# ljubobratovicrelja/tensor-truth

Measured on AMD Instinct MI355X. Metric: queries/sec (embed+top-k+rerank) over 10M x 1024 corpus, higher is better.
Workload: dtype bf16

## Files before the change

### tensor-truth_amd/csrc/encoder.h

```cpp
#pragma once
#include "common.h"

enum { TT_EPI_BIAS = 0, TT_EPI_GELU = 1, TT_EPI_RESIDUAL = 2, TT_EPI_TANH = 3, TT_EPI_QKV = 4,
       TT_EPI_VT = 5 ,
       TT_EPI_SCAN = 6  };

struct GemmParams {
    const uint16_t* A;
    const uint16_t* W;
    const float* bias;
    const uint16_t* residual;
    uint16_t* C;
    uint16_t* vt;
    int M, N, K, lda, ldc, ldr, ldvt, vt_col0;
    const float* a_scale;
    const float* w_scale;
    int fp8;
    uint8_t* C8;
    float c8_inv_scale;
    int nt_store;
    int sn;
    int xp;
    int32_t* scan_cnt;
    float* scan_scores;
    int32_t* scan_idx;
    int scan_cap;
    int32_t scan_idx_base;
    float* scan_dense;
    int scan_dense_stride;
    int scan_tile_stride;
    int scan_rows;
    int x3;
    int ldw;
    int c_lo_off;
    float* C32;
    const float* res32;
    const uint16_t* res_planes;
    int res_lo_off;
    uint16_t* vt_lo;
    int x3_zero_lo;
    int xc;
    const uint8_t* a_scales;
    const uint8_t* w_scales;
    uint8_t* c_scales;
#if TT_DIAG
    int lnf;
    const float* lnf_rows;
    const float* lnf_c0;
    const float* lnf_c1;
    float* lnf_part;
#endif
};
int tt_scan_gemm_launch(const uint16_t* corpus, int64_t rows, int dim, const uint16_t* queries256, const float* thr256,
                        int32_t* cnt, float* cand_scores, int32_t* cand_idx, int cap, int32_t idx_base, hipStream_t st);
int tt_scan_gemm_sample_launch(const uint16_t* corpus, int tiles, int tile_stride, int dim, const uint16_t* queries256, const float* thr256,
// ... 98 lines not shown
```

### tensor-truth_amd/csrc/gemm.hip

```cpp
#include "common.h"
#include <type_traits>

#include "encoder.h"
#include "f16c.h"

namespace {

constexpr int BM = 128, BN = 128, BK = 64;
constexpr int kGemmThreads = 256;
constexpr int kTileBytes = BM * BK * 2;
constexpr int kStageBytes = 2 * kTileBytes;
constexpr int kGemmLds = 2 * kStageBytes;

__device__ __forceinline__ f32x2 gelu_erf2(f32x2 x) {
    const f32x2 u = f32x2{fabsf(x.x), fabsf(x.y)};
    f32x2 q = u * -9.697845371e-07f + 4.016999810e-05f;
    q = q * u + -7.211678312e-04f;
    q = q * u + 7.490924560e-03f;
    q = q * u + -5.142170191e-02f;
    q = q * u + -4.614778757e-01f;
    q = q * u + -1.149914980e+00f;
    q = q * u + -1.000091195e+00f;
    const f32x2 e = f32x2{__builtin_amdgcn_exp2f(q.x), __builtin_amdgcn_exp2f(q.y)};
    const f32x2 r = f32x2{fmaxf(x.x, 0.f), fmaxf(x.y, 0.f)};
// ... 920 lines not shown
                    }
                }
        }
}

#define TT_SLOT_END()                                         \
    do {                                                      \
        __builtin_amdgcn_sched_barrier(0);                    \
        __builtin_amdgcn_s_barrier();                         \
        __builtin_amdgcn_sched_barrier(0);                    \
    } while (0)

typedef int v8i __attribute__((ext_vector_type(8)));
struct Frag2 { ex8 lo, hi; };
__device__ __forceinline__ f32x4 mfma_fp8(const ex8& a0, const ex8& a1, const ex8& b0, const ex8& b1, f32x4 c) {
    const v8i a = __builtin_bit_cast(v8i, Frag2{a0, a1});
    const v8i b = __builtin_bit_cast(v8i, Frag2{b0, b1});
    return __builtin_amdgcn_mfma_scale_f32_16x16x128_f8f6f4(a, b, c, 0, 0, 0, 0x7F7F7F7F, 0, 0x7F7F7F7F);
}

constexpr int kXcScaleOff = kLds3;
constexpr int kLdsXc = kLds3 + 2 * 8192;
__device__ __forceinline__ void glds4(const void* base, uint32_t voff, uint32_t lds_addr) {
    asm volatile("s_mov_b32 m0, %2\n\ts_nop 0\n\tglobal_load_lds_dword %0, %1"
                 :: "v"(voff), "s"(base), "s"(lds_addr) : "memory", "m0");
}
template <int OA, int OB>
__device__ __forceinline__ f32x4 mfma_fp8_scaled(const ex8& a0, const ex8& a1, const ex8& b0, const ex8& b1, f32x4 c, uint32_t scale_a,
                                                 uint32_t scale_b) {
    const v8i a = __builtin_bit_cast(v8i, Frag2{a0, a1});
    const v8i b = __builtin_bit_cast(v8i, Frag2{b0, b1});
    return __builtin_amdgcn_mfma_scale_f32_16x16x128_f8f6f4(a, b, c, 0, 0, OA, (int)scale_a, OB, (int)scale_b);
}
template <int N, class F>
__device__ __forceinline__ void static_for(F&& f) {
    if constexpr (N > 0) {
        static_for<N - 1>(f);
        f(std::integral_constant<int, N - 1>{});
    }
}

template <int EPI, int SLOTS, bool FP8 = false, bool X3 = false, bool XC = false, bool RP = false>
__global__ __launch_bounds__(kThreads3, 2) void gemm_kernel_v3(GemmParams p) {
    static_assert(!(FP8 && X3), "split-bf16 operands are bf16");
    static_assert(!XC || (!FP8 && !X3 && kF16), "f16c operands: the fp16 instantiation, no other operand mode");
    constexpr int ES = FP8 ? 1 : 2;
    extern __shared__ __attribute__((aligned(16))) char smem[];
    const int tid = threadIdx.x;
    const int lane = tid & 63;
    const int wave = __builtin_amdgcn_readfirstlane(tid >> 6);
    const int wm = wave >> 2, wn = wave & 3;

    const int mt_n = p.M / BM3, nt_n = (p.N + BN3 - 1) / BN3;
    int L = blockIdx.x;
    {
        const int nwg = gridDim.x;
        if ((nwg & 7) == 0) L = (L & 7) * (nwg >> 3) + (L >> 3);
    }
    const int SN = p.sn > 0 ? p.sn : (nt_n < 4 ? nt_n : 4);
    const int SM = 32 / SN > 0 ? 32 / SN : 1;
    const int per_super = SM * SN;
    const int supers_n = (nt_n + SN - 1) / SN;
    const int sidx = L / per_super, widx = L % per_super;
    const int tm = (sidx / supers_n) * SM + widx / SN;
    const int tn = (sidx % supers_n) * SN + widx % SN;
    if (tm >= mt_n || tn >= nt_n) return;
    int m0_nominal = tm * BM3;
    if constexpr (EPI == TT_EPI_SCAN) {
        if (p.scan_tile_stride > 1) m0_nominal *= p.scan_tile_stride;
        if (p.scan_rows && m0_nominal + BM3 > p.scan_rows) m0_nominal = p.scan_rows - BM3;
    }
    const int m0 = m0_nominal, n0 = tn * BN3;
    const int nk1 = p.K * ES / 128;
    constexpr int TB = X3 ? 64 : 128;
    const int nk = X3 ? 2 * nk1 : (XC ? 2 * nk1 : nk1);
    auto tile_a = [&](int t) { return t; };
    auto tile_w = [&](int t) { return t; };

    f32x4 acc[2][2][2][4];
#pragma unroll
    for (int a = 0; a < 2; ++a)
#pragma unroll
        for (int b = 0; b < 2; ++b)
#pragma unroll
            for (int c = 0; c < 2; ++c)
#pragma unroll
                for (int d = 0; d < 4; ++d) acc[a][b][c][d] = f32x4{0.f, 0.f, 0.f, 0.f};

    const int frow = lane & 15, fchk = lane >> 4, sw = (frow >> 1) & 7;
    const int off0 = frow * 128 + ((fchk ^ sw) << 4);
    const int off1 = frow * 128 + (((4 + fchk) ^ sw) << 4);
    const int a_row0 = wm * 64 * 128;
    const int w_row0 = wn * 32 * 128;

    uint32_t voffA[2], voffW[2];
#pragma unroll
    for (int j = 0; j < 2; ++j) {
        const int r = 16 * wave + 8 * j + (lane >> 3);
        const int chunk = (lane & 7) ^ ((r >> 1) & 7);
        const uint32_t coff = X3 ? (chunk < 4 ? (uint32_t)chunk * 16u : (uint32_t)p.K * 2u + (uint32_t)(chunk - 4) * 16u) : (uint32_t)chunk * 16u;
        voffA[j] = (uint32_t)r * (uint32_t)p.lda * (uint32_t)ES + coff;
        const int wr = (X3 && n0 + (r >> 5) * 64 + 64 > p.N) ? 0 : w_row_of(r);
        voffW[j] = (uint32_t)wr * (uint32_t)(p.ldw ? p.ldw : p.K) * (uint32_t)ES + coff;
    }

    unsigned long long* dbg0 = reinterpret_cast<unsigned long long*>(p.vt);
    auto cstamp = [&](int slot) {
        if constexpr (SLOTS == 46) {
            if ((int)blockIdx.x == (p.xp >> 20) && tid == 0 && dbg0) dbg0[20 + slot] = __builtin_amdgcn_s_memtime();
            if ((slot == 0 || slot == 3) && tid == 0 && dbg0) {
                unsigned long long* rec = dbg0 + 256 + (size_t)blockIdx.x * 4;
                rec[slot == 0 ? 0 : 1] = __builtin_amdgcn_s_memtime();
                if (slot == 0)
                    rec[2] = ((unsigned long long)__builtin_amdgcn_s_getreg(20 | (31 << 11)) << 32) |
                             (unsigned long long)__builtin_amdgcn_s_getreg(4 | (31 << 11));
            }
        }
    };
    constexpr bool kResLds = (EPI == TT_EPI_RESIDUAL) && !X3 && !XC;
    uint32_t voffR[2] = {0u, 0u};
    if constexpr (kResLds) {
#pragma unroll
        for (int j = 0; j < 2; ++j) {
            const int r16 = 8 * j + (lane >> 3);
            const int c = (lane & 7) ^ ((r16 >> 1) & 7);
            voffR[j] = (uint32_t)r16 * (uint32_t)p.ldr * 2u + (uint32_t)(c * 16);
        }
    }
    auto stage_res = [&](int part) {
        if constexpr (kResLds) {
#pragma unroll
            for (int od = 0; od < 2; ++od) {
                const char* base = reinterpret_cast<const char*>(
                    p.residual + (size_t)(m0 + (part >> 1) * 128 + wm * 64 + ((part & 1) * 2 + od) * 16) * p.ldr + n0 + wn * 64);
                const unsigned long long b64 = reinterpret_cast<unsigned long long>(base);
                const unsigned int blo = __builtin_amdgcn_readfirstlane((unsigned int)b64);
                const unsigned int bhi = __builtin_amdgcn_readfirstlane((unsigned int)(b64 >> 32));
                base = reinterpret_cast<const char*>(((unsigned long long)bhi << 32) | blo);
                char* dst = smem + (res_slot(part) + 4 * od) * kHalf + 2048 * wave;
                const uint32_t lds_dst = (uint32_t)(uintptr_t)(__attribute__((address_space(3))) char*)dst;
#pragma unroll
                for (int j = 0; j < 2; ++j) glds16(base, voffR[j], lds_dst + 1024 * j);
            }
        }
    };

    cstamp(0);
    if constexpr (EPI == TT_EPI_SCAN) {
        if (tid == 0) *reinterpret_cast<int*>(smem + kScanHitOff) = 0;
        if ((p.xp & 0x10000) && lane == 0) *reinterpret_cast<int*>(smem + kScanHitOff + wave * 1024) = 0;
    }
    if (wave == 0) {
        uint32_t boff = lane * 16;
        if constexpr (X3) {
            const uint32_t last = (uint32_t)((p.N - n0 < BN3 ? p.N - n0 : BN3) * 4 - 16);
            boff = boff < last ? boff : last;
        }
        glds16(p.bias + n0, boff, (uint32_t)(uintptr_t)(__attribute__((address_space(3))) char*)smem + kBiasOff);
    }
    if constexpr (FP8 && EPI != TT_EPI_VT) {
        if (wave == 1) glds16(p.a_scale + m0, lane * 16, (uint32_t)(uintptr_t)(__attribute__((address_space(3))) char*)smem + kScaleOff);
        if (wave == 2) glds16(p.w_scale + n0, lane * 16, (uint32_t)(uintptr_t)(__attribute__((address_space(3))) char*)smem + kScaleOff + 1024);
    }
#if TT_DIAG
    if constexpr (!FP8 && !X3 && !XC && (EPI == TT_EPI_BIAS || EPI == TT_EPI_GELU || EPI == TT_EPI_RESIDUAL)) {
        if (p.lnf) {
            const uint32_t l0 = (uint32_t)(uintptr_t)(__attribute__((address_space(3))) char*)smem;
            if (wave == 1) glds16(p.lnf_c0 + n0, lane * 16, l0 + kScaleOff);
            if (wave == 2 && p.lnf == 2) glds16(p.lnf_c1 + n0, lane * 16, l0 + kScaleOff + 1024);
            if (wave == 3) glds16(p.lnf_rows + (size_t)m0 * 2, lane * 16, l0 + kScaleOff + 2048);
            if (wave == 4) glds16(p.lnf_rows + (size_t)(m0 + 128) * 2, lane * 16, l0 + kScaleOff + 3072);
        }
    }
#endif
    stage_half<0, ES>(p, smem, 0, 0, 0, wave, voffA, m0, n0, TB);
    stage_half<1, ES>(p, smem, 0, 0, 0, wave, voffW, m0, n0, TB);
    stage_half<1, ES>(p, smem, 1, 0, 0, wave, voffW, m0, n0, TB);
    stage_half<0, ES>(p, smem, 1, 0, 0, wave, voffA, m0, n0, TB);
    if (nk > 1) {
        stage_half<0, ES>(p, smem, 0, 1, tile_a(1), wave, voffA, m0, n0, TB);
        stage_half<1, ES>(p, smem, 0, 1, tile_w(1), wave, voffW, m0, n0, TB);
    }
    if (nk > 1) {
        asm volatile("s_waitcnt vmcnt(6)" ::: "memory");
    } else {
        asm volatile("s_waitcnt vmcnt(0)" ::: "memory");
    }
    TT_SLOT_END();
    cstamp(1);
    const bool late = wave >= 4;
    if (late) TT_SLOT_END();

    ex8 xf[4][2], wf0[2][2], wf1[2][2];

    auto read_a = [&](const char* base) {
#pragma unroll
        for (int mt = 0; mt < 4; ++mt) {
            xf[mt][0] = *reinterpret_cast<const ex8*>(base + a_row0 + mt * 2048 + off0);
            xf[mt][1] = *reinterpret_cast<const ex8*>(base + a_row0 + mt * 2048 + off1);
        }
    };
    auto read_w = [&](ex8(&wf)[2][2], const char* base) {
#pragma unroll
        for (int nt = 0; nt < 2; ++nt) {
            wf[nt][0] = *reinterpret_cast<const ex8*>(base + w_row0 + nt * 2048 + off0);
            wf[nt][1] = *reinterpret_cast<const ex8*>(base + w_row0 + nt * 2048 + off1);
        }
    };
    uint32_t sa_reg[2] = {0u, 0u}, sw_reg = 0u;
    const int sa_off = (wm * 16 + frow) * 16 + fchk * 4;
    const int sw_off = 1024 + (wn * 16 + frow) * 16 + fchk * 4;
    auto stage_scales = [&](int t) {
        if constexpr (XC) {
            const int u = t - nk1 + (wave >> 1), nks = nk1 >> 1;
            const uint8_t* src = (wave & 1) ? p.w_scales + ((size_t)(n0 >> 8) * nk1 + u) * 1024
                                            : p.a_scales + ((size_t)(m0 >> 8) * nks + (u >= nks ? u - nks : u)) * 1024;
            const unsigned long long b64 = reinterpret_cast<unsigned long long>(src);
            const unsigned int blo = __builtin_amdgcn_readfirstlane((unsigned int)b64);
            const unsigned int bhi = __builtin_amdgcn_readfirstlane((unsigned int)(b64 >> 32));
            const uint32_t dst = (uint32_t)(uintptr_t)(__attribute__((address_space(3))) char*)smem + kXcScaleOff +
                                 (((t - nk1) >> 2) & 1) * 8192 + wave * 1024;
            glds16(reinterpret_cast<const void*>(((unsigned long long)bhi << 32) | blo), (uint32_t)lane * 16u, dst);
        }
    };
    constexpr bool vblk = (EPI == TT_EPI_VT);
    auto mma = [&](f32x4(&c)[2][4], const ex8(&wf)[2][2]) {
        __builtin_amdgcn_s_setprio(1);
        if constexpr (FP8) {
#pragma unroll
            for (int nt = 0; nt < 2; ++nt)
#pragma unroll
                for (int mt = 0; mt < 4; ++mt) {
                    if constexpr (vblk) c[nt][mt] = mfma_fp8(xf[mt][0], xf[mt][1], wf[nt][0], wf[nt][1], c[nt][mt]);
                    else c[nt][mt] = mfma_fp8(wf[nt][0], wf[nt][1], xf[mt][0], xf[mt][1], c[nt][mt]);
                }
        } else if constexpr (X3) {
#pragma unroll
            for (int term = 0; term < 3; ++term) {
                const int sa = term == 2 ? 1 : 0, sw = term == 1 ? 1 : 0;
#pragma unroll
                for (int nt = 0; nt < 2; ++nt)
#pragma unroll
                    for (int mt = 0; mt < 4; ++mt) {
                        if constexpr (vblk) c[nt][mt] = TT_MFMA_16x16x32(xf[mt][sa], wf[nt][sw], c[nt][mt]);
                        else c[nt][mt] = TT_MFMA_16x16x32(wf[nt][sw], xf[mt][sa], c[nt][mt]);
                    }
            }
        } else if constexpr (vblk) {
#pragma unroll
            for (int ss = 0; ss < 2; ++ss)
#pragma unroll
                for (int nt = 0; nt < 2; ++nt)
#pragma unroll
                    for (int mt = 0; mt < 4; ++mt)
                        c[nt][mt] = TT_MFMA_16x16x32(xf[mt][ss], wf[nt][ss], c[nt][mt]);
        } else {
#pragma unroll
            for (int ss = 0; ss < 2; ++ss)
#pragma unroll
                for (int nt = 0; nt < 2; ++nt)
#pragma unroll
                    for (int mt = 0; mt < 4; ++mt)
                        c[nt][mt] = TT_MFMA_16x16x32(wf[nt][ss], xf[mt][ss], c[nt][mt]);
        }
        __builtin_amdgcn_s_setprio(0);
    };
    auto mma8 = [&](f32x4(&c)[2][4], const ex8(&wf)[2][2], uint32_t sa, uint32_t sw, auto qnc) {
        if constexpr (XC) {
            constexpr int QN = decltype(qnc)::value;
            __builtin_amdgcn_s_setprio(1);
            static_for<2>([&](auto ntc) {
                static_for<4>([&](auto mtc) {
                    constexpr int nt = decltype(ntc)::value, mt = decltype(mtc)::value;
                    if constexpr (vblk) c[nt][mt] = mfma_fp8_scaled<mt, QN * 2 + nt>(xf[mt][0], xf[mt][1], wf[nt][0], wf[nt][1], c[nt][mt], sa, sw);
                    else c[nt][mt] = mfma_fp8_scaled<QN * 2 + nt, mt>(wf[nt][0], wf[nt][1], xf[mt][0], xf[mt][1], c[nt][mt], sw, sa);
                });
            });
            __builtin_amdgcn_s_setprio(0);
        }
    };
    unsigned long long* dbg = reinterpret_cast<unsigned long long*>(p.vt);
    int dbg_i = 0;
    auto stamp = [&](int t) {
        if constexpr (SLOTS == 46) {
            if ((int)blockIdx.x == (p.xp >> 20) && t == 6 && (lane == 0) && dbg) {
                __builtin_amdgcn_sched_barrier(0);
                dbg[wave * 32 + dbg_i] = __builtin_amdgcn_s_memtime();
                ++dbg_i;
                __builtin_amdgcn_sched_barrier(0);
            }
        }
    };
    auto wait_n = [&](int n) {
        if (n == 8) asm volatile("s_waitcnt vmcnt(8) lgkmcnt(0)" ::: "memory");
        else if (n == 6) asm volatile("s_waitcnt vmcnt(6) lgkmcnt(0)" ::: "memory");
        else if (n == 9) asm volatile("s_waitcnt vmcnt(9) lgkmcnt(0)" ::: "memory");
        else if (n == 7) asm volatile("s_waitcnt vmcnt(7) lgkmcnt(0)" ::: "memory");
        else asm volatile("s_waitcnt vmcnt(0) lgkmcnt(0)" ::: "memory");
        TT_SLOT_END();
    };
#if TT_DIAG
    const int eabl = (p.xp & 0x80000) ? ((p.xp >> 4) & 15) : 0;
#else
    constexpr int eabl = 0;
#endif
    auto tile4 = [&](int t, auto bufc, auto f8c) {
        constexpr int B = decltype(bufc)::value;
        constexpr bool F8T = XC && decltype(f8c)::value;
        const bool dma_on = !((eabl & 1) && t >= 2), rd_on = !((eabl & 2) && t >= 2);
        const bool more1 = t + 1 < nk && dma_on, more2 = t + 2 < nk && dma_on;
        const int sc_la = (XC && t + 1 >= nk1 && t + 1 < nk && ((t + 1 - nk1) & 3) == 0) ? 1 : 0;
        const int sc_lb = (XC && t + 2 >= nk1 && t + 2 < nk && ((t + 2 - nk1) & 3) == 0) ? 1 : 0;
        const char* sbuf = smem + kXcScaleOff + (((t - nk1) >> 2) & 1) * 8192 + ((t - nk1) & 3) * 2048;
        stamp(t);
        if (more1) {
            stage_half<1, ES>(p, smem, 1, B ^ 1, tile_w(t + 1), wave, voffW, m0, n0, TB);
            stage_half<0, ES>(p, smem, 1, B ^ 1, tile_a(t + 1), wave, voffA, m0, n0, TB);
        } else if (kResLds) {
            stage_res(1);
        }
        stamp(t);
        if (rd_on) {
            read_a(smem + slot_off(0, 0, B));
            read_w(wf0, smem + slot_off(1, 0, B));
            read_w(wf1, smem + slot_off(1, 1, B));
        }
        if constexpr (F8T) {
            sa_reg[0] = *reinterpret_cast<const uint32_t*>(sbuf + sa_off);
            sw_reg = *reinterpret_cast<const uint32_t*>(sbuf + sw_off);
        }
        stamp(t);
        if (SLOTS == 46) asm volatile("s_waitcnt lgkmcnt(0)" ::: "memory");
        stamp(t);
        wait_n((t + 1 < nk || kResLds) ? 8 + sc_la : 0);
        stamp(t);
        if constexpr (F8T) {
            mma8(acc[0][0], wf0, sa_reg[0], sw_reg, std::integral_constant<int, 0>{});
            mma8(acc[0][1], wf1, sa_reg[0], sw_reg, std::integral_constant<int, 1>{});
        } else {
            mma(acc[0][0], wf0);
            mma(acc[0][1], wf1);
        }
        stamp(t);
        TT_SLOT_END();
        stamp(t);
        if (more2) {
            stage_half<0, ES>(p, smem, 0, B, tile_a(t + 2), wave, voffA, m0, n0, TB);
            stage_half<1, ES>(p, smem, 0, B, tile_w(t + 2), wave, voffW, m0, n0, TB);
            if (sc_lb) stage_scales(t + 2);
        } else if (kResLds) {
            stage_res(B == 0 ? 0 : 2);
        }
        stamp(t);
        if (rd_on) read_a(smem + slot_off(0, 1, B));
        if constexpr (F8T) sa_reg[1] = *reinterpret_cast<const uint32_t*>(sbuf + 512 + sa_off);
        stamp(t);
        if (SLOTS == 46) asm volatile("s_waitcnt lgkmcnt(0)" ::: "memory");
        stamp(t);
        wait_n((t + 2 < nk || kResLds) ? 6 + sc_lb : 0);
        stamp(t);
        if constexpr (F8T) {
            mma8(acc[1][1], wf1, sa_reg[1], sw_reg, std::integral_constant<int, 1>{});
            mma8(acc[1][0], wf0, sa_reg[1], sw_reg, std::integral_constant<int, 0>{});
        } else {
            mma(acc[1][1], wf1);
            mma(acc[1][0], wf0);
        }
        stamp(t);
        TT_SLOT_END();
        stamp(t);
    };

    if constexpr (XC) {
        for (int t = 0; t < nk1; t += 2) {
            tile4(t, std::integral_constant<int, 0>{}, std::false_type{});
            tile4(t + 1, std::integral_constant<int, 1>{}, std::false_type{});
        }
        for (int t = nk1; t < nk; t += 2) {
            tile4(t, std::integral_constant<int, 0>{}, std::true_type{});
            tile4(t + 1, std::integral_constant<int, 1>{}, std::true_type{});
        }
    } else {
        for (int t = 0; t < nk; t += 2) {
            tile4(t, std::integral_constant<int, 0>{}, std::false_type{});
            if (t + 1 < nk) tile4(t + 1, std::integral_constant<int, 1>{}, std::false_type{});
        }
    }
    cstamp(2);
    if (!late) TT_SLOT_END();
    stage_res(3);

    if constexpr (X3) {
        if (n0 + wn * 64 >= p.N) return;
    }
    if constexpr (vblk) {
#pragma unroll
        for (int qm = 0; qm < 2; ++qm)
#pragma unroll
            for (int qn = 0; qn < 2; ++qn)
                gemm_epilogue_vt<2, 4, FP8, X3>(p, acc[qm][qn], m0 + qm * 128 + wm * 64, n0 + wn * 64 + qn * 32, lane);
    } else if constexpr (X3) {
        epilogue_x3<EPI, RP>(p, acc, smem, kBiasOff, m0, n0, wm, wn, lane);
    } else if constexpr (XC && EPI == TT_EPI_RESIDUAL) {
        epilogue_x3<EPI>(p, acc, smem, kBiasOff, m0, n0, wm, wn, lane);
    } else if constexpr (XC && EPI == TT_EPI_GELU) {
        epilogue_xc<EPI>(p, acc, smem, kBiasOff, m0, n0, wm, wn, lane);
    } else if constexpr (XC && EPI == TT_EPI_BIAS) {
        if (p.c_lo_off) epilogue_h2(p, acc, smem, kBiasOff, m0, n0, wm, wn, lane);
        else epilogue_all<EPI, true, false>(p, acc, smem, kBiasOff, kScaleOff, m0, n0, wm, wn, wave, lane, false, NoNext{});
    } else if constexpr (EPI == TT_EPI_QKV) {
#pragma unroll
        for (int qm = 0; qm < 2; ++qm)
#pragma unroll
            for (int qn = 0; qn < 2; ++qn)
                gemm_epilogue_wide<EPI, 2, 4>(p, acc[qm][qn], m0 + qm * 128 + wm * 64, n0 + wn * 64 + qn * 32, lane);
    } else if constexpr (EPI == TT_EPI_SCAN) {
        if (p.scan_dense) scan_sample_epilogue(p, acc, tm, wm, wn, lane);
        else if (p.xp & 0x10000) scan_filter_epilogue<2>(p, acc, smem, kBiasOff, m0, wm, wn, lane);
        else scan_filter_epilogue<1>(p, acc, smem, kBiasOff, m0, wm, wn, lane);
    } else if constexpr (SLOTS == 47) {
#pragma unroll
        for (int qm = 0; qm < 2; ++qm)
#pragma unroll
            for (int qn = 0; qn < 2; ++qn)
                gemm_epilogue_wide<EPI, 2, 4, true>(p, acc[qm][qn], m0 + qm * 128 + wm * 64, n0 + wn * 64 + qn * 32, lane);
    } else {
        epilogue_all<EPI, true, FP8>(p, acc, smem, kBiasOff, kScaleOff, m0, n0, wm, wn, wave, lane, false, NoNext{}, kScaleOff, kScaleOff + 2048);
    }
    if constexpr (SLOTS == 46) {
        asm volatile("s_waitcnt vmcnt(0)" ::: "memory");
        cstamp(3);
    }
}

template <int EPI, bool FP8 = false, bool STAMP = false>
__global__ __launch_bounds__(kThreads3, 2) void gemm_kernel_p(GemmParams p, int nwg) {
    constexpr int ES = FP8 ? 1 : 2;
    extern __shared__ __attribute__((aligned(16))) char smem[];
    const int tid = threadIdx.x;
    const int lane = tid & 63;
    const int wave = __builtin_amdgcn_readfirstlane(tid >> 6);
    const int wm = wave >> 2, wn = wave & 3;

    const int mt_n = p.M / BM3, nt_n = p.N / BN3;
    const int SN = p.sn > 0 ? p.sn : (nt_n < 4 ? nt_n : 4);
    const int SM = 32 / SN > 0 ? 32 / SN : 1;
    const int per_super = SM * SN;
    const int supers_n = (nt_n + SN - 1) / SN;
    const int nk = p.K * ES / 128;
    auto decode = [&](int v, int& m0, int& n0) {
        const int L = (v & 7) * (nwg >> 3) + (v >> 3);
        const int sidx = L / per_super, widx = L % per_super;
        const int tm = (sidx / supers_n) * SM + widx / SN;
        const int tn = (sidx % supers_n) * SN + widx % SN;
        int mm = tm * BM3;
        if constexpr (EPI == TT_EPI_SCAN) {
            if (p.scan_rows && mm + BM3 > p.scan_rows) mm = p.scan_rows - BM3;
        }
        m0 = __builtin_amdgcn_readfirstlane(mm);
        n0 = __builtin_amdgcn_readfirstlane(tn * BN3);
        return tm < mt_n && tn < nt_n;
    };
    auto next_valid = [&](int v, int& m0, int& n0) {
        for (v += gridDim.x; v < nwg; v += gridDim.x)
// ... 172 lines not shown
        const bool align = (p.xp & 4) == 0;
        if (align && !late) TT_SLOT_END();

        int lane_e = lane;
        asm volatile("" : "+v"(lane_e));
        if constexpr (EPI == TT_EPI_SCAN)
            scan_filter_epilogue<2>(p, acc, smem, kBiasOff + bpar * 1024, m0, wm, wn, lane_e);
        else
            epilogue_all<EPI, false, FP8>(p, acc, smem, kBiasOff + bpar * 1024, kScaleOff + bpar * 2048, m0, n0, wm, wn, wave, lane_e,
                                          false, NoNext{}, kScaleOff + bpar * 1024, kScaleOff + 2048 + bpar * 2048);
        pstamp(101);
        ++tile_no;
        if (!has_next) {
            if (!align && !late) TT_SLOT_END();
            break;
        }
        if (align && late) TT_SLOT_END();
        v = vn; m0 = m1; n0 = n1; bpar ^= 1; first = false;
        vn = next_valid(v, m1, n1);
        has_next = vn < nwg;
    }
}
#undef TT_SLOT_END
}

inline int super_sn(int nt_n) {
    static const int env = TT_DIAG_ENV_INT("TT_GEMM_SN", 0);
    int sn = env > 0 ? env : 4;
    if (sn > nt_n) sn = nt_n;
    while (32 % sn) --sn;
    return sn;
}

inline bool small_grid_v1() {
    static const bool on = TT_DIAG_ENV_INT("TT_GEMM_SMALL_V1", 1) != 0;
    return on;
}

template <int EPI>
int launch_fp8(const GemmParams& p, hipStream_t st) {
    if constexpr (EPI == TT_EPI_BIAS || EPI == TT_EPI_GELU || EPI == TT_EPI_VT || EPI == TT_EPI_RESIDUAL) {
        const int nk = p.K / 128;
        if (EPI == TT_EPI_RESIDUAL && (!p.residual || p.ldr % 8)) {
            tt_set_error("gemm fp8: residual epilogue without residual");
            return TT_E_INVALID;
        }
        if (p.M % v3::BM3 || p.N % v3::BN3 || p.K % 128 || nk < 2 || (nk & 1) || p.ldc % 8 || p.lda % 16 || !p.a_scale || !p.w_scale) {
            tt_set_error("gemm fp8: M=%d N=%d K=%d must be multiples of 256/256/256 with row / column scales", p.M, p.N, p.K);
            return TT_E_UNSUPPORTED;
        }
        const int mt_n = p.M / v3::BM3, nt_n = p.N / v3::BN3;
        const int SN = super_sn(nt_n), SM = 32 / SN;
        const int supers = ((mt_n + SM - 1) / SM) * ((nt_n + SN - 1) / SN);
        int blocks = supers * SM * SN;
        blocks = (blocks + 7) / 8 * 8;
        TT_SET_MAX_LDS((v3::gemm_kernel_v3<EPI, 4, true>), v3::kLds3);
        {
            TtProfScope prof(TT_K_GEMM, st);
            GemmParams q = p;
            q.sn = SN;
            hipLaunchKernelGGL((v3::gemm_kernel_v3<EPI, 4, true>), dim3(blocks), dim3(v3::kThreads3), v3::kLds3, st, q);
        }
        TT_CHECK_LAUNCH();
        return TT_OK;
    } else {
        tt_set_error("gemm fp8: epilogue %d has no fp8 form", EPI);
// ... 508 lines not shown

template <int EPI>
int launch(const GemmParams& p, hipStream_t st) {
    if constexpr (!kF16) if (p.fp8) return launch_fp8<EPI>(p, st);
    static const bool trace = TT_DIAG_ENV_INT("TT_GEMM_TRACE", 0) == 1;
    if (trace) fprintf(stderr, "gemm launch<%d> M=%d N=%d K=%d lda=%d ldc=%d ldr=%d\n", EPI, p.M, p.N, p.K, p.lda, p.ldc, p.ldr);
    static const int variant = TT_DIAG_ENV_INT("TT_GEMM_VARIANT", 5);
    const bool small_grid = EPI != TT_EPI_VT && (long long)(p.M / v3::BM3) * (p.N / v3::BN3) < 128 && small_grid_v1();
    if (variant >= 4 && !small_grid && p.M % v3::BM3 == 0 && p.N % v3::BN3 == 0 && p.ldc % 8 == 0 &&
        (EPI != TT_EPI_RESIDUAL || (p.ldr % 8 == 0 && (p.K / BK) % 2 == 0))) {
        const int mt_n = p.M / v3::BM3, nt_n = p.N / v3::BN3;
        const int SN = super_sn(nt_n), SM = 32 / SN;
        const int supers = ((mt_n + SM - 1) / SM) * ((nt_n + SN - 1) / SN);
        int blocks = supers * SM * SN;
        blocks = (blocks + 7) / 8 * 8;
        static const int xp = TT_DIAG_ENV_INT("TT_GEMM_XP", 0);
        if constexpr (EPI == TT_EPI_GELU || EPI == TT_EPI_BIAS) {
            const int cus = tt_cu_count_cached() / 8 * 8;
            if (variant == 5 && (EPI == TT_EPI_GELU || (xp & 1)) && (p.K / BK) % 2 == 0 && p.K / BK >= 2 && blocks > cus && cus >= 8) {
                constexpr int kLdsP = v3::kLds3 + (TT_DIAG ? 2048 : 0);
                TT_SET_MAX_LDS(v3::gemm_kernel_p<EPI>, kLdsP);
                {
                    TtProfScope prof(TT_K_GEMM, st);
                    GemmParams q = p;
                    q.sn = SN;
                    q.xp = xp;
                    hipLaunchKernelGGL(v3::gemm_kernel_p<EPI>, dim3(cus), dim3(v3::kThreads3), kLdsP, st, q, blocks);
                }
                TT_CHECK_LAUNCH();
                return TT_OK;
            }
        }
        auto kern = v3::gemm_kernel_v3<EPI, 4>;
#if TT_DIAG
        if constexpr (EPI == TT_EPI_BIAS) {
            static const int abl = TT_DIAG_ENV_INT("TT_GEMM_ABLATE", 0);
            if (abl == 8) {
                const int cus8 = tt_cu_count_cached() / 8 * 8;
                TT_SET_MAX_LDS((v3::gemm_kernel_p<EPI, false, true>), v3::kLds3);
                GemmParams q8 = p;
                q8.sn = SN;
                q8.xp = xp;
                hipLaunchKernelGGL((v3::gemm_kernel_p<EPI, false, true>), dim3(cus8), dim3(v3::kThreads3), v3::kLds3, st, q8, blocks);
                TT_CHECK_LAUNCH();
                return TT_OK;
            }
            if (abl == 6) kern = v3::gemm_kernel_v3<EPI, 46>;
            if (abl == 7) kern = v3::gemm_kernel_v3<EPI, 47>;
            if (abl == 6 || abl == 7) TT_CHECK_HIP(hipFuncSetAttribute(reinterpret_cast<const void*>(kern), hipFuncAttributeMaxDynamicSharedMemorySize, v3::kLds3));
        }
#endif
        TT_SET_MAX_LDS((v3::gemm_kernel_v3<EPI, 4>), v3::kLds3);
        GemmParams q = p;
        static const int nts = TT_DIAG_ENV_INT("TT_GEMM_NT_STORE", 1);
        q.nt_store = nts;
        q.sn = SN;
        static const bool a0 = TT_DIAG_ENV_INT("TT_GEMM_DEBUG_A0", 0) == 1;
        if (a0) q.xp |= 0x20000;
        static const bool head_major = TT_DIAG_ENV_INT("TT_GEMM_HEAD_MAJOR", 0) == 1;
        if (head_major) q.xp |= 0x40000;
        static const int stamp_block = TT_DIAG_ENV_INT("TT_GEMM_STAMP_BLOCK", 0);
        q.xp |= stamp_block << 20;
        static const int energy = TT_DIAG_ENV_INT("TT_GEMM_ENERGY", 0);
        if (energy) q.xp |= 0x80000 | ((energy & 15) << 4);
        {
            TtProfScope prof(TT_K_GEMM, st);
            hipLaunchKernelGGL(kern, dim3(blocks), dim3(v3::kThreads3), v3::kLds3, st, q);
        }
        TT_CHECK_LAUNCH();
        return TT_OK;
    }
    if constexpr (EPI == TT_EPI_VT) {
        tt_set_error("gemm: internal V^T epilogue needs the 256x256 kernel");
        return TT_E_UNSUPPORTED;
    }
    const int mt_n = p.M / BM, nt_n = p.N / BN;
    const int SN = nt_n < 8 ? nt_n : 8, SM = 8;
    const int supers = ((mt_n + SM - 1) / SM) * ((nt_n + SN - 1) / SN);
    int blocks = supers * SM * SN;
    blocks = (blocks + 7) / 8 * 8;
    static const int staged16 = TT_DIAG_ENV_INT("TT_GEMM_STAGED16", 1);
    if (staged16 && staged_enabled() && (long long)mt_n * nt_n <= (staged16 > 1 ? staged16 : tt_cu_count_cached()) && p.K % 64 == 0) {
        TT_SET_MAX_LDS((gemm_staged_kernel<EPI, false>), kStagedLds);
        {
            TtProfScope prof(TT_K_GEMM, st);
            hipLaunchKernelGGL((gemm_staged_kernel<EPI, false>), dim3(blocks), dim3(kStagedThreads), kStagedLds, st, p);
        }
        TT_CHECK_LAUNCH();
        return TT_OK;
    }
    auto kern = gemm_kernel<EPI>;
    TT_SET_MAX_LDS(kern, kGemmLds);
    {
        TtProfScope prof(TT_K_GEMM, st);
        hipLaunchKernelGGL(kern, dim3(blocks), dim3(kGemmThreads), kGemmLds, st, p);
    }
    TT_CHECK_LAUNCH();
    return TT_OK;
}

// ... 49 lines not shown
    if ((p.lda % 8) || (p.ldc % 4) || !p.A || !p.W || !p.C || !p.bias) {
        tt_set_error("gemm: bad leading dimension / null pointer");
        return TT_E_INVALID;
    }
    if (skinny_shape(p)) {
        switch (epilogue) {
            case TT_EPI_BIAS: return launch_skinny<TT_EPI_BIAS>(p, st);
            case TT_EPI_GELU: return launch_skinny<TT_EPI_GELU>(p, st);
            case TT_EPI_RESIDUAL:
                if (!p.residual || p.ldr % 4) { tt_set_error("gemm: residual epilogue without residual"); return TT_E_INVALID; }
                return launch_skinny<TT_EPI_RESIDUAL>(p, st);
            case TT_EPI_TANH: return launch_skinny<TT_EPI_TANH>(p, st);
            case TT_EPI_QKV:
                if (!p.vt || p.vt_col0 % 16) { tt_set_error("gemm: qkv epilogue without vt"); return TT_E_INVALID; }
                return launch_skinny<TT_EPI_QKV>(p, st);
            default: tt_set_error("gemm: unknown epilogue %d", epilogue); return TT_E_INVALID;
        }
    }
    if (p.M % BM || p.N % BN || p.K % BK || p.K <= 0) {
        tt_set_error("gemm: M=%d N=%d K=%d must be multiples of %d/%d/%d (or M a multiple of 64 up to 256)", p.M, p.N, p.K, BM, BN, BK);
        return TT_E_UNSUPPORTED;
    }
    switch (epilogue) {
        case TT_EPI_BIAS: return launch<TT_EPI_BIAS>(p, st);
        case TT_EPI_GELU: return launch<TT_EPI_GELU>(p, st);
        case TT_EPI_RESIDUAL:
            if (!p.residual) { tt_set_error("gemm: residual epilogue without residual"); return TT_E_INVALID; }
            return launch<TT_EPI_RESIDUAL>(p, st);
        case TT_EPI_TANH: return launch<TT_EPI_TANH>(p, st);
        case TT_EPI_QKV: {
            if (!p.vt) { tt_set_error("gemm: qkv epilogue without vt"); return TT_E_INVALID; }
            static const int variant = TT_DIAG_ENV_INT("TT_GEMM_VARIANT", 5);
            const int nv = p.N - p.vt_col0;
            static const int split = TT_DIAG_ENV_INT("TT_GEMM_QKV_SPLIT", 1);
            const bool small_grid = (long long)(p.M / v3::BM3) * (p.N / v3::BN3) < 128 && small_grid_v1();
            if (variant >= 3 && split && !small_grid && p.M % v3::BM3 == 0 && p.vt_col0 % v3::BN3 == 0 && nv % v3::BN3 == 0 &&
                nv > 0 && p.ldc % 8 == 0 && p.ldvt % 8 == 0) {
                GemmParams a = p;
                a.N = p.vt_col0;
                if (int rc = launch<TT_EPI_BIAS>(a, st)) return rc;
                GemmParams b = p;
                b.W = p.W + (size_t)p.vt_col0 * p.K;
                b.bias = p.bias + p.vt_col0;
                b.N = nv;
                b.vt_col0 = 0;
                return launch<TT_EPI_VT>(b, st);
            }
            return launch<TT_EPI_QKV>(p, st);
        }
        default: tt_set_error("gemm: unknown epilogue %d", epilogue); return TT_E_INVALID;
    }
}

#ifndef TT_SCAN_PERSIST_DEFAULT
#define TT_SCAN_PERSIST_DEFAULT 1
#endif
int tt_scan_gemm_sample_launch(const uint16_t* corpus, int tiles, int tile_stride, int dim, const uint16_t* queries256, const float* thr256,
                               float* dense, int dense_stride, hipStream_t st) {
    if (tiles <= 0) return TT_OK;
    if constexpr (kF16) { tt_set_error("scan gemm: the corpus is bf16 (bf16 instantiation only)"); return TT_E_UNSUPPORTED; }
    else
    if (dim % 128 || dim <= 0 || tile_stride < 1 || !dense || dense_stride < tiles * 8 || (int64_t)tiles * tile_stride * v3::BM3 > INT32_MAX) {
        tt_set_error("scan gemm sample: tiles=%d stride=%d dim=%d dense_stride=%d", tiles, tile_stride, dim, dense_stride);
        return TT_E_UNSUPPORTED;
    }
    GemmParams p{};
    p.A = corpus;
    p.W = queries256;
    p.bias = thr256;
    p.M = tiles * v3::BM3;
// ... 70 lines not shown
```

Measured before the change: 110.2.

## Walk multiple GEMM tiles per workgroup in the v3 bf16 kernel

```diff
diff --git a/tensor-truth_amd/csrc/encoder.h b/tensor-truth_amd/csrc/encoder.h
--- a/tensor-truth_amd/csrc/encoder.h
+++ b/tensor-truth_amd/csrc/encoder.h
@@ -21,6 +21,7 @@
     int nt_store;
     int sn;
     int xp;
+    int walk, walk_rounds, walk_slots;
     int32_t* scan_cnt;
     float* scan_scores;
     int32_t* scan_idx;
diff --git a/tensor-truth_amd/csrc/gemm.hip b/tensor-truth_amd/csrc/gemm.hip
--- a/tensor-truth_amd/csrc/gemm.hip
+++ b/tensor-truth_amd/csrc/gemm.hip
@@ -984,8 +984,8 @@
     }
 }
 
-template <int EPI, int SLOTS, bool FP8 = false, bool X3 = false, bool XC = false, bool RP = false>
-__global__ __launch_bounds__(kThreads3, 2) void gemm_kernel_v3(GemmParams p) {
+template <int EPI, int SLOTS, bool FP8, bool X3, bool XC, bool RP>
+__device__ __forceinline__ void gemm_tile_v3(const GemmParams& p, const int L, const int bias_off) {
     static_assert(!(FP8 && X3), "split-bf16 operands are bf16");
     static_assert(!XC || (!FP8 && !X3 && kF16), "f16c operands: the fp16 instantiation, no other operand mode");
     constexpr int ES = FP8 ? 1 : 2;
@@ -996,18 +996,12 @@
     const int wm = wave >> 2, wn = wave & 3;
 
     const int mt_n = p.M / BM3, nt_n = (p.N + BN3 - 1) / BN3;
-    int L = blockIdx.x;
-    {
-        const int nwg = gridDim.x;
-        if ((nwg & 7) == 0) L = (L & 7) * (nwg >> 3) + (L >> 3);
-    }
-    const int SN = p.sn > 0 ? p.sn : (nt_n < 4 ? nt_n : 4);
-    const int SM = 32 / SN > 0 ? 32 / SN : 1;
-    const int per_super = SM * SN;
-    const int supers_n = (nt_n + SN - 1) / SN;
-    const int sidx = L / per_super, widx = L % per_super;
-    const int tm = (sidx / supers_n) * SM + widx / SN;
-    const int tn = (sidx % supers_n) * SN + widx % SN;
+    const int SN = p.sn, lsn = __builtin_ctz((unsigned)SN), SM = 32 >> lsn;
+    const int supers_n = (nt_n + SN - 1) >> lsn;
+    const int sidx = L >> 5, widx = L & 31;
+    const int srow = (int)((unsigned)sidx / (unsigned)supers_n);
+    const int tm = srow * SM + (widx >> lsn);
+    const int tn = (sidx - srow * supers_n) * SN + (widx & (SN - 1));
     if (tm >= mt_n || tn >= nt_n) return;
     int m0_nominal = tm * BM3;
     if constexpr (EPI == TT_EPI_SCAN) {
@@ -1053,7 +1047,7 @@
         if constexpr (SLOTS == 46) {
             if ((int)blockIdx.x == (p.xp >> 20) && tid == 0 && dbg0) dbg0[20 + slot] = __builtin_amdgcn_s_memtime();
             if ((slot == 0 || slot == 3) && tid == 0 && dbg0) {
-                unsigned long long* rec = dbg0 + 256 + (size_t)blockIdx.x * 4;
+                unsigned long long* rec = dbg0 + 256 + (size_t)L * 4;
                 rec[slot == 0 ? 0 : 1] = __builtin_amdgcn_s_memtime();
                 if (slot == 0)
                     rec[2] = ((unsigned long long)__builtin_amdgcn_s_getreg(20 | (31 << 11)) << 32) |
@@ -1100,7 +1094,7 @@
             const uint32_t last = (uint32_t)((p.N - n0 < BN3 ? p.N - n0 : BN3) * 4 - 16);
             boff = boff < last ? boff : last;
         }
-        glds16(p.bias + n0, boff, (uint32_t)(uintptr_t)(__attribute__((address_space(3))) char*)smem + kBiasOff);
+        glds16(p.bias + n0, boff, (uint32_t)(uintptr_t)(__attribute__((address_space(3))) char*)smem + bias_off);
     }
     if constexpr (FP8 && EPI != TT_EPI_VT) {
         if (wave == 1) glds16(p.a_scale + m0, lane * 16, (uint32_t)(uintptr_t)(__attribute__((address_space(3))) char*)smem + kScaleOff);
@@ -1344,14 +1338,14 @@
             for (int qn = 0; qn < 2; ++qn)
                 gemm_epilogue_vt<2, 4, FP8, X3>(p, acc[qm][qn], m0 + qm * 128 + wm * 64, n0 + wn * 64 + qn * 32, lane);
     } else if constexpr (X3) {
-        epilogue_x3<EPI, RP>(p, acc, smem, kBiasOff, m0, n0, wm, wn, lane);
+        epilogue_x3<EPI, RP>(p, acc, smem, bias_off, m0, n0, wm, wn, lane);
     } else if constexpr (XC && EPI == TT_EPI_RESIDUAL) {
-        epilogue_x3<EPI>(p, acc, smem, kBiasOff, m0, n0, wm, wn, lane);
+        epilogue_x3<EPI>(p, acc, smem, bias_off, m0, n0, wm, wn, lane);
     } else if constexpr (XC && EPI == TT_EPI_GELU) {
-        epilogue_xc<EPI>(p, acc, smem, kBiasOff, m0, n0, wm, wn, lane);
+        epilogue_xc<EPI>(p, acc, smem, bias_off, m0, n0, wm, wn, lane);
     } else if constexpr (XC && EPI == TT_EPI_BIAS) {
-        if (p.c_lo_off) epilogue_h2(p, acc, smem, kBiasOff, m0, n0, wm, wn, lane);
-        else epilogue_all<EPI, true, false>(p, acc, smem, kBiasOff, kScaleOff, m0, n0, wm, wn, wave, lane, false, NoNext{});
+        if (p.c_lo_off) epilogue_h2(p, acc, smem, bias_off, m0, n0, wm, wn, lane);
+        else epilogue_all<EPI, true, false>(p, acc, smem, bias_off, kScaleOff, m0, n0, wm, wn, wave, lane, false, NoNext{});
     } else if constexpr (EPI == TT_EPI_QKV) {
 #pragma unroll
         for (int qm = 0; qm < 2; ++qm)
@@ -1360,8 +1354,8 @@
                 gemm_epilogue_wide<EPI, 2, 4>(p, acc[qm][qn], m0 + qm * 128 + wm * 64, n0 + wn * 64 + qn * 32, lane);
     } else if constexpr (EPI == TT_EPI_SCAN) {
         if (p.scan_dense) scan_sample_epilogue(p, acc, tm, wm, wn, lane);
-        else if (p.xp & 0x10000) scan_filter_epilogue<2>(p, acc, smem, kBiasOff, m0, wm, wn, lane);
-        else scan_filter_epilogue<1>(p, acc, smem, kBiasOff, m0, wm, wn, lane);
+        else if (p.xp & 0x10000) scan_filter_epilogue<2>(p, acc, smem, bias_off, m0, wm, wn, lane);
+        else scan_filter_epilogue<1>(p, acc, smem, bias_off, m0, wm, wn, lane);
     } else if constexpr (SLOTS == 47) {
 #pragma unroll
         for (int qm = 0; qm < 2; ++qm)
@@ -1369,11 +1363,57 @@
             for (int qn = 0; qn < 2; ++qn)
                 gemm_epilogue_wide<EPI, 2, 4, true>(p, acc[qm][qn], m0 + qm * 128 + wm * 64, n0 + wn * 64 + qn * 32, lane);
     } else {
-        epilogue_all<EPI, true, FP8>(p, acc, smem, kBiasOff, kScaleOff, m0, n0, wm, wn, wave, lane, false, NoNext{}, kScaleOff, kScaleOff + 2048);
+        epilogue_all<EPI, true, FP8>(p, acc, smem, bias_off, kScaleOff, m0, n0, wm, wn, wave, lane, false, NoNext{}, kScaleOff, kScaleOff + 2048);
     }
     if constexpr (SLOTS == 46) {
         asm volatile("s_waitcnt vmcnt(0)" ::: "memory");
         cstamp(3);
+    }
+}
+
+template <int EPI, int SLOTS, bool FP8 = false, bool X3 = false, bool XC = false, bool RP = false, bool WALK = false>
+__global__ __launch_bounds__(kThreads3, 2) void gemm_kernel_v3(GemmParams p) {
+    const int nwg = gridDim.x;
+    if constexpr (!WALK) {
+        int L = blockIdx.x;
+        if ((nwg & 7) == 0) L = (L & 7) * (nwg >> 3) + (L >> 3);
+        gemm_tile_v3<EPI, SLOTS, FP8, X3, XC, RP>(p, L, kBiasOff);
+    } else {
+        static_assert(!FP8 && !X3 && !XC && (EPI == TT_EPI_BIAS || EPI == TT_EPI_VT || EPI == TT_EPI_RESIDUAL), "walked forms");
+        const int x = blockIdx.x & 7, u = blockIdx.x >> 3;
+        const int T = p.walk, R = p.walk_rounds;
+        const int walkers = (R + T - 1) / T * 32;
+        int slot = x * p.walk_slots, count = 1;
+        if (u < walkers) {
+            const int g = u >> 5;
+            slot += g * T * 32 + (u & 31);
+            count = R - g * T < T ? R - g * T : T;
+        } else {
+            slot += R * 32 + (u - walkers);
+        }
+        typedef unsigned long long __attribute__((may_alias)) Word;
+        typedef const __attribute__((address_space(4))) Word* KernArg;
+        static_assert(sizeof(GemmParams) % sizeof(Word) == 0, "GemmParams is copied in 8-byte words");
+#pragma unroll 1
+        for (int t = 0; t < count; ++t) {
+            KernArg kp = (KernArg)__builtin_amdgcn_kernarg_segment_ptr();
+            asm volatile("" : "+s"(kp));
+            GemmParams q;
+#pragma unroll
+            for (size_t i = 0; i < sizeof(GemmParams) / sizeof(Word); ++i) reinterpret_cast<Word*>(&q)[i] = kp[i];
+#define TT_KARG_GLOBAL(field, T)                                                                                             \
+    q.field = (T*)*(__attribute__((address_space(1))) T* const __attribute__((address_space(4)))*)(                          \
+        (const __attribute__((address_space(4))) char*)kp + offsetof(GemmParams, field))
+            TT_KARG_GLOBAL(bias, const float);
+            TT_KARG_GLOBAL(C, uint16_t);
+            TT_KARG_GLOBAL(C8, uint8_t);
+            TT_KARG_GLOBAL(vt, uint16_t);
+#undef TT_KARG_GLOBAL
+#if TT_DIAG
+            q.lnf = 0;
+#endif
+            gemm_tile_v3<EPI, SLOTS, FP8, X3, XC, RP>(q, slot + t * 32, kBiasOff + (t & 1) * 1024);
+        }
     }
 }
 
@@ -1612,6 +1652,8 @@
     return sn;
 }
 
+constexpr int kWalkTiles = 4;
+
 inline bool small_grid_v1() {
     static const bool on = TT_DIAG_ENV_INT("TT_GEMM_SMALL_V1", 1) != 0;
     return on;
@@ -2186,9 +2228,11 @@
             }
         }
         auto kern = v3::gemm_kernel_v3<EPI, 4>;
+        [[maybe_unused]] int ablate = 0;
 #if TT_DIAG
         if constexpr (EPI == TT_EPI_BIAS) {
             static const int abl = TT_DIAG_ENV_INT("TT_GEMM_ABLATE", 0);
+            ablate = abl;
             if (abl == 8) {
                 const int cus8 = tt_cu_count_cached() / 8 * 8;
                 TT_SET_MAX_LDS((v3::gemm_kernel_p<EPI, false, true>), v3::kLds3);
@@ -2217,9 +2261,35 @@
         q.xp |= stamp_block << 20;
         static const int energy = TT_DIAG_ENV_INT("TT_GEMM_ENERGY", 0);
         if (energy) q.xp |= 0x80000 | ((energy & 15) << 4);
+        int grid = blocks;
+        if constexpr (EPI == TT_EPI_BIAS || EPI == TT_EPI_VT || EPI == TT_EPI_RESIDUAL) {
+            static const int T = TT_DIAG_ENV_INT("TT_GEMM_WALK", kWalkTiles);
+            static const int mask = TT_DIAG_ENV_INT("TT_GEMM_WALK_MASK", (1 << TT_EPI_BIAS) | (1 << TT_EPI_RESIDUAL) | (1 << TT_EPI_VT));
+            const int slots = blocks / 8, rounds = slots / 32 - 1;
+            bool walk = T > 1 && ((mask >> EPI) & 1) && rounds >= 2 && ablate != 7;
+#if TT_DIAG
+            if (p.lnf) walk = false;
+#endif
+            if (walk) {
+                q.walk = T;
+                q.walk_rounds = rounds;
+                q.walk_slots = slots;
+                grid = 8 * ((rounds + T - 1) / T * 32 + slots - 32 * rounds);
+                kern = v3::gemm_kernel_v3<EPI, 4, false, false, false, false, true>;
+                TT_SET_MAX_LDS((v3::gemm_kernel_v3<EPI, 4, false, false, false, false, true>), v3::kLds3);
+#if TT_DIAG
+                if constexpr (EPI == TT_EPI_BIAS) {
+                    if (ablate == 6) {
+                        kern = v3::gemm_kernel_v3<EPI, 46, false, false, false, false, true>;
+                        TT_CHECK_HIP(hipFuncSetAttribute(reinterpret_cast<const void*>(kern), hipFuncAttributeMaxDynamicSharedMemorySize, v3::kLds3));
+                    }
+                }
+#endif
+            }
+        }
         {
             TtProfScope prof(TT_K_GEMM, st);
-            hipLaunchKernelGGL(kern, dim3(blocks), dim3(v3::kThreads3), v3::kLds3, st, q);
+            hipLaunchKernelGGL(kern, dim3(grid), dim3(v3::kThreads3), v3::kLds3, st, q);
         }
         TT_CHECK_LAUNCH();
         return TT_OK;
```

Measured after the change: 110.5, median of 6. No clear change (+0.3%).

## Fuse split QKV GEMM launches into one kernel with per-tile V-transpose path

Applied to the files above, without the earlier changes.

```diff
diff --git a/tensor-truth_amd/csrc/gemm.hip b/tensor-truth_amd/csrc/gemm.hip
--- a/tensor-truth_amd/csrc/gemm.hip
+++ b/tensor-truth_amd/csrc/gemm.hip
@@ -976,6 +976,7 @@
     const v8i b = __builtin_bit_cast(v8i, Frag2{b0, b1});
     return __builtin_amdgcn_mfma_scale_f32_16x16x128_f8f6f4(a, b, c, 0, 0, OA, (int)scale_a, OB, (int)scale_b);
 }
+
 template <int N, class F>
 __device__ __forceinline__ void static_for(F&& f) {
     if constexpr (N > 0) {
@@ -1167,8 +1168,11 @@
             glds16(reinterpret_cast<const void*>(((unsigned long long)bhi << 32) | blo), (uint32_t)lane * 16u, dst);
         }
     };
-    constexpr bool vblk = (EPI == TT_EPI_VT);
-    auto mma = [&](f32x4(&c)[2][4], const ex8(&wf)[2][2]) {
+    constexpr bool vblk_ct = (EPI == TT_EPI_VT);
+    constexpr bool kQkvTiles = (EPI == TT_EPI_QKV) && !FP8 && !X3 && !XC;
+    const bool v_tile = kQkvTiles && (p.xp & 0x8) && n0 >= p.vt_col0;
+    auto mma = [&](f32x4(&c)[2][4], const ex8(&wf)[2][2], auto vtc) {
+        constexpr bool vblk = vblk_ct || decltype(vtc)::value;
         __builtin_amdgcn_s_setprio(1);
         if constexpr (FP8) {
 #pragma unroll
@@ -1216,7 +1220,7 @@
             static_for<2>([&](auto ntc) {
                 static_for<4>([&](auto mtc) {
                     constexpr int nt = decltype(ntc)::value, mt = decltype(mtc)::value;
-                    if constexpr (vblk) c[nt][mt] = mfma_fp8_scaled<mt, QN * 2 + nt>(xf[mt][0], xf[mt][1], wf[nt][0], wf[nt][1], c[nt][mt], sa, sw);
+                    if constexpr (vblk_ct) c[nt][mt] = mfma_fp8_scaled<mt, QN * 2 + nt>(xf[mt][0], xf[mt][1], wf[nt][0], wf[nt][1], c[nt][mt], sa, sw);
                     else c[nt][mt] = mfma_fp8_scaled<QN * 2 + nt, mt>(wf[nt][0], wf[nt][1], xf[mt][0], xf[mt][1], c[nt][mt], sw, sa);
                 });
             });
@@ -1248,7 +1252,7 @@
 #else
     constexpr int eabl = 0;
 #endif
-    auto tile4 = [&](int t, auto bufc, auto f8c) {
+    auto tile4 = [&](int t, auto bufc, auto f8c, auto vtc) {
         constexpr int B = decltype(bufc)::value;
         constexpr bool F8T = XC && decltype(f8c)::value;
         const bool dma_on = !((eabl & 1) && t >= 2), rd_on = !((eabl & 2) && t >= 2);
@@ -1282,8 +1286,8 @@
             mma8(acc[0][0], wf0, sa_reg[0], sw_reg, std::integral_constant<int, 0>{});
             mma8(acc[0][1], wf1, sa_reg[0], sw_reg, std::integral_constant<int, 1>{});
         } else {
-            mma(acc[0][0], wf0);
-            mma(acc[0][1], wf1);
+            mma(acc[0][0], wf0, vtc);
+            mma(acc[0][1], wf1, vtc);
         }
         stamp(t);
         TT_SLOT_END();
@@ -1307,8 +1311,8 @@
             mma8(acc[1][1], wf1, sa_reg[1], sw_reg, std::integral_constant<int, 1>{});
             mma8(acc[1][0], wf0, sa_reg[1], sw_reg, std::integral_constant<int, 0>{});
         } else {
-            mma(acc[1][1], wf1);
-            mma(acc[1][0], wf0);
+            mma(acc[1][1], wf1, vtc);
+            mma(acc[1][0], wf0, vtc);
         }
         stamp(t);
         TT_SLOT_END();
@@ -1317,17 +1321,25 @@
 
     if constexpr (XC) {
         for (int t = 0; t < nk1; t += 2) {
-            tile4(t, std::integral_constant<int, 0>{}, std::false_type{});
-            tile4(t + 1, std::integral_constant<int, 1>{}, std::false_type{});
+            tile4(t, std::integral_constant<int, 0>{}, std::false_type{}, std::false_type{});
+            tile4(t + 1, std::integral_constant<int, 1>{}, std::false_type{}, std::false_type{});
         }
         for (int t = nk1; t < nk; t += 2) {
-            tile4(t, std::integral_constant<int, 0>{}, std::true_type{});
-            tile4(t + 1, std::integral_constant<int, 1>{}, std::true_type{});
+            tile4(t, std::integral_constant<int, 0>{}, std::true_type{}, std::false_type{});
+            tile4(t + 1, std::integral_constant<int, 1>{}, std::true_type{}, std::false_type{});
         }
     } else {
-        for (int t = 0; t < nk; t += 2) {
-            tile4(t, std::integral_constant<int, 0>{}, std::false_type{});
-            if (t + 1 < nk) tile4(t + 1, std::integral_constant<int, 1>{}, std::false_type{});
+        auto k_loop = [&](auto vtc) {
+            for (int t = 0; t < nk; t += 2) {
+                tile4(t, std::integral_constant<int, 0>{}, std::false_type{}, vtc);
+                if (t + 1 < nk) tile4(t + 1, std::integral_constant<int, 1>{}, std::false_type{}, vtc);
+            }
+        };
+        if constexpr (kQkvTiles) {
+            if (v_tile) k_loop(std::true_type{});
+            else k_loop(std::false_type{});
+        } else {
+            k_loop(std::false_type{});
         }
     }
     cstamp(2);
@@ -1337,7 +1349,7 @@
     if constexpr (X3) {
         if (n0 + wn * 64 >= p.N) return;
     }
-    if constexpr (vblk) {
+    if constexpr (vblk_ct) {
 #pragma unroll
         for (int qm = 0; qm < 2; ++qm)
 #pragma unroll
@@ -1353,11 +1365,21 @@
         if (p.c_lo_off) epilogue_h2(p, acc, smem, kBiasOff, m0, n0, wm, wn, lane);
         else epilogue_all<EPI, true, false>(p, acc, smem, kBiasOff, kScaleOff, m0, n0, wm, wn, wave, lane, false, NoNext{});
     } else if constexpr (EPI == TT_EPI_QKV) {
-#pragma unroll
-        for (int qm = 0; qm < 2; ++qm)
-#pragma unroll
-            for (int qn = 0; qn < 2; ++qn)
-                gemm_epilogue_wide<EPI, 2, 4>(p, acc[qm][qn], m0 + qm * 128 + wm * 64, n0 + wn * 64 + qn * 32, lane);
+        if (v_tile) {
+#pragma unroll
+            for (int qm = 0; qm < 2; ++qm)
+#pragma unroll
+                for (int qn = 0; qn < 2; ++qn)
+                    gemm_epilogue_vt<2, 4, false, false>(p, acc[qm][qn], m0 + qm * 128 + wm * 64, n0 + wn * 64 + qn * 32, lane);
+        } else if (p.xp & 0x8) {
+            epilogue_all<TT_EPI_BIAS, true, false>(p, acc, smem, kBiasOff, kScaleOff, m0, n0, wm, wn, wave, lane, false, NoNext{});
+        } else {
+#pragma unroll
+            for (int qm = 0; qm < 2; ++qm)
+#pragma unroll
+                for (int qn = 0; qn < 2; ++qn)
+                    gemm_epilogue_wide<EPI, 2, 4>(p, acc[qm][qn], m0 + qm * 128 + wm * 64, n0 + wn * 64 + qn * 32, lane);
+        }
     } else if constexpr (EPI == TT_EPI_SCAN) {
         if (p.scan_dense) scan_sample_epilogue(p, acc, tm, wm, wn, lane);
         else if (p.xp & 0x10000) scan_filter_epilogue<2>(p, acc, smem, kBiasOff, m0, wm, wn, lane);
@@ -2335,10 +2357,15 @@
             if (!p.vt) { tt_set_error("gemm: qkv epilogue without vt"); return TT_E_INVALID; }
             static const int variant = TT_DIAG_ENV_INT("TT_GEMM_VARIANT", 5);
             const int nv = p.N - p.vt_col0;
-            static const int split = TT_DIAG_ENV_INT("TT_GEMM_QKV_SPLIT", 1);
+            static const int split = TT_DIAG_ENV_INT("TT_GEMM_QKV_SPLIT", 2);
             const bool small_grid = (long long)(p.M / v3::BM3) * (p.N / v3::BN3) < 128 && small_grid_v1();
             if (variant >= 3 && split && !small_grid && p.M % v3::BM3 == 0 && p.vt_col0 % v3::BN3 == 0 && nv % v3::BN3 == 0 &&
                 nv > 0 && p.ldc % 8 == 0 && p.ldvt % 8 == 0) {
+                if (split == 2) {
+                    GemmParams q = p;
+                    q.xp |= 0x8;
+                    return launch<TT_EPI_QKV>(q, st);
+                }
                 GemmParams a = p;
                 a.N = p.vt_col0;
                 if (int rc = launch<TT_EPI_BIAS>(a, st)) return rc;
```

New measurement: 113.5 before, 114.0 after (median of 6 runs). About the same (+0.5%).
